# infil00p/openbts-ttsou

Measured on AMD Instinct MI355X. Metric: Mbursts/s (156.25-sym @ 4 sps) demod+detect, higher is better.
Workload: dtype f32

## Files before the change

openbts-ttsou_amd/csrc/trxsig_corr.h:

```cpp
#pragma once
#include "trxsig_dev.h"

namespace {

template <int SPS>
struct CorrGeom {
  static constexpr int NL = 36 * SPS;
  static constexpr int NC = (NL + 15) / 16;
  static constexpr int FRONT = 8 * SPS;
  static constexpr int WPAD0 = NC * 16 + 15 * SPS + 1;
  static constexpr int WPAD = ((WPAD0 + 15) / 32) * 32 + 16;
  static constexpr int H = (5 * SPS + 1 > 12) ? 5 * SPS + 1 : 12;
  static constexpr int NS = 2 * H + 1;
  static constexpr int NE = 20 * SPS;
  static constexpr int NEQ = (NE + 15) / 16;
  static constexpr int NPAIR = (NS + 2) / 2;
};
template <typename T>
__device__ __forceinline__ T &rec_slot(T *rec, int Bpad, int s, int b) { return rec[2 * ((size_t)(s >> 1) * Bpad + b) + (s & 1)]; }

template <int N>
__device__ __forceinline__ float add_row_shl(float acc, float v) {
  float r;
  if (N == 0) asm volatile("v_add_f32 %0, %1, %2" : "=v"(r) : "v"(v), "v"(acc));
  else asm volatile("v_add_f32_dpp %0, %1, %2 row_shl:%3 row_mask:0xf bank_mask:0xf bound_ctrl:1"
                    : "=v"(r) : "v"(v), "v"(acc), "n"(N));
  return r;
}
template <int SPS, int I>
__device__ __forceinline__ float energy_chain_step(float acc, const float (&nrm)[CorrGeom<SPS>::NEQ]) {
  if constexpr (I < CorrGeom<SPS>::NE) {
    acc = add_row_shl<I % 16>(acc, nrm[I / 16]);
    return energy_chain_step<SPS, I + 1>(acc, nrm);
  } else {
    return acc;
  }
}
template <int SPS, int I>
__device__ __forceinline__ float energy_chain(float acc, const float (&nrm)[CorrGeom<SPS>::NEQ]) {
  asm volatile("s_nop 1");
  return energy_chain_step<SPS, I>(acc, nrm);
}

template <int SPS>
struct CorrIn {
  typedef CorrGeom<SPS> G;
  static constexpr int NW = (CorrGeom<SPS>::NL + 15) / 16;
  cx w[NW];
  cx e[CorrGeom<SPS>::NEQ];
  int b;
  bool live, good;
  __device__ __forceinline__ void stage_window(cx *W, int r) const {
#pragma unroll
    for (int i = 0; i < NW; i++) {
      const int q = r + 16 * i;
      if (q < G::NL) W[G::FRONT + q] = w[i];
    }
  }
  __device__ __forceinline__ void stage_norms(float *ef, int r) const {
#pragma unroll
    for (int q = 0; q < G::NEQ; q++) {
      const int i = r + 16 * q;
      if (i < G::NE) ef[i] = norm2(e[q]);
    }
  }
};

template <int SPS>
__device__ __forceinline__ void corr_issue(CorrIn<SPS> &in, int b, int B, int r, const cx *__restrict__ samples,
                                           const int32_t *__restrict__ offset, const int32_t *__restrict__ length) {
  typedef CorrGeom<SPS> G;
  in.b = b;
  in.live = b < B;
  int off = 0, len = 0;
  if (in.live) { off = offset[b]; len = length[b]; }
  in.good = in.live && (off >= 0) && (len >= 92 * SPS) && (len <= 157 * SPS) && (len % SPS == 0);
  const cx *x = samples + (in.good ? off : 0);
#pragma unroll
  for (int i = 0; i < CorrIn<SPS>::NW; i++) {
    const int q = r + 16 * i;
    in.w[i] = (in.good && q < G::NL) ? x[56 * SPS + q] : mk(0, 0);
  }
#pragma unroll
  for (int q = 0; q < G::NEQ; q++) {
    const int i = r + 16 * q;
    in.e[q] = (in.good && i < G::NE) ? x[i] : mk(0, 0);
  }
}

template <int SPS, bool REC, bool EFIRST = false, unsigned TAPCLS = TRX_TAPS_GENERIC, typename IN = CorrIn<SPS>>
__device__ __forceinline__ void corr_round(const IN &in, cx *W, float4 *E, int lane, int r, const cx (&tap)[16],
                                           cx *__restrict__ rec, int Bpad, int &M_out, float &energy_out) {
  typedef CorrGeom<SPS> G;
  auto stage_norms = [&] { in.stage_norms(reinterpret_cast<float *>(E), r); };
  auto sum_norms = [&] {
    float energy = 0.0f;
#pragma unroll
    for (int i4 = 0; i4 < (G::NE + 3) / 4; i4++) {
      const float4 e = E[i4];
      energy = energy + e.x;
      if (4 * i4 + 1 < G::NE) energy = energy + e.y;
      if (4 * i4 + 2 < G::NE) energy = energy + e.z;
      if (4 * i4 + 3 < G::NE) energy = energy + e.w;
    }
    return energy;
  };
  float energy = 0.0f;
  if (EFIRST) {
    stage_norms();
    wave_lds_fence();
    energy = sum_norms();
    asm volatile("" : "+v"(energy));
    wave_lds_fence();
  }
  for (int q = r; q < G::FRONT; q += 16) W[q] = mk(0, 0);
  for (int q = G::FRONT + G::NL + r; q < G::WPAD; q += 16) W[q] = mk(0, 0);
  in.stage_window(W, r);
  if (!EFIRST) stage_norms();
  wave_lds_fence();
  if (!EFIRST) energy = sum_norms();

  float bestP = 0.0f;
  int bestT = -1;
  cx cval[G::NC];
  constexpr int CG = (SPS == 4) ? TRX_CORR_CG : 1;
  constexpr int UPC = 16 / SPS;
  constexpr int NU = UPC * (CG - 1) + 16;
#pragma unroll
  for (int c0 = 0; c0 < G::NC; c0 += CG) {
    cx sv[NU];
#pragma unroll
    for (int u = 0; u < NU; u++) sv[u] = W[r + 16 * c0 + SPS * u];
#pragma unroll
    for (int cc = 0; cc < CG; cc++) {
      if (c0 + cc < G::NC) {
        cx acc = mk(0, 0);
#pragma unroll
        for (int k = 15; k >= 0; k--) acc = cadd(acc, cmul_tap(sv[UPC * cc + k], tap[k], (TAPCLS >> (2 * k)) & 3));
        cval[c0 + cc] = acc;
      }
    }
  }
  wave_lds_fence();
#pragma unroll
  for (int c = 0; c < G::NC; c++) {
    const int t = r + 16 * c;
    if (t < G::NL) {
      W[t] = cval[c];
      const float p = norm2(cval[c]);
      if (p > bestP) { bestP = p; bestT = t; }
    }
  }
#pragma unroll
  for (int m = 1; m < 16; m <<= 1) {
    const float oP = __shfl_xor(bestP, m, 64);
    const int oT = __shfl_xor(bestT, m, 64);
    const bool take = (oP > bestP) || (oP == bestP && oT >= 0 && (bestT < 0 || oT < bestT));
    if (take) { bestP = oP; bestT = oT; }
  }
  wave_lds_fence();

  M_out = bestT;
  energy_out = energy;
  if (REC && in.live) {
    const int M = bestT;
    auto slot = [&](int s) {
      cx v = mk(0, 0);
      if (s < G::NS) {
        const int lag = M - G::H + s;
        if (lag >= 0 && lag < G::NL) v = W[lag];
      } else if (s == G::NS) {
        v = mk(__int_as_float(in.good ? M : -2), energy);
      }
      return v;
    };
    for (int j = r; j < G::NPAIR; j += 16) {
      const cx a = slot(2 * j), c = slot(2 * j + 1);
      reinterpret_cast<float4 *>(rec)[(size_t)j * Bpad + in.b] = make_float4(a.r, a.i, c.r, c.i);
    }
  }
  wave_lds_fence();
  (void)lane;
}


inline unsigned tap_classes(const TrxTables *hT, int tsc) {
  unsigned m = 0;
  for (int k = 0; k < 16; k++) {
    const trx_c32 a = hT->mid_ctap[tsc][k];
    const unsigned c = (a.r == 1.0f || a.r == -1.0f) ? 1u : ((a.i == 1.0f || a.i == -1.0f) ? 2u : 0u);
    m |= c << (2 * k);
  }
  return m;
}

}
```

openbts-ttsou_amd/csrc/trxsig_dev.h:

```cpp
#pragma once
#include <hip/hip_runtime.h>
#include <hip/hip_fp16.h>
#include <stdint.h>

#include <type_traits>

#include "trxsig_tables.h"
#include "trxsig_launch.h"

#ifndef TRX_CORR_CG
#define TRX_CORR_CG 3
#endif
#ifndef TRX_CORR_WPS
#define TRX_CORR_WPS 1
#endif
#ifndef TRX_CORR_ROUNDS
#define TRX_CORR_ROUNDS 1
#endif
#ifndef TRX_DEMOD_WAVES
#define TRX_DEMOD_WAVES 4
#endif

namespace {

typedef trx_c32 cx;

__device__ __forceinline__ cx mk(float r, float i) { cx z; z.r = r; z.i = i; return z; }
__device__ __forceinline__ cx cmul(cx x, cx a) { return mk(x.r * a.r - x.i * a.i, x.r * a.i + x.i * a.r); }
__device__ __forceinline__ cx cmul_sum(cx x, cx a, float nai) { return mk(x.r * a.r + x.i * nai, x.r * a.i + x.i * a.r); }
__device__ __forceinline__ float neg_opaque(float v) {
  float r = -v;
  asm volatile("" : "+v"(r));
  return r;
}
__device__ __forceinline__ cx cmul_sum(cx x, cx a) { return cmul_sum(x, a, neg_opaque(a.i)); }
__device__ __forceinline__ cx cmulr(cx x, float a) { return mk(x.r * a, x.i * a); }
__device__ __forceinline__ cx cadd(cx x, cx a) { return mk(x.r + a.r, x.i + a.i); }
__device__ __forceinline__ float norm2(cx x) { return x.i * x.i + x.r * x.r; }
__device__ __forceinline__ cx cinv(cx x) { float n = norm2(x); return mk(x.r / n, -x.i / n); }
__device__ __forceinline__ cx cdiv(cx x, cx a) { return cmul(x, cinv(a)); }

template <int CTRL>
__device__ __forceinline__ float dpp_f(float v) {
  return __int_as_float(__builtin_amdgcn_update_dpp(0, __float_as_int(v), CTRL, 0xf, 0xf, true));
}
template <int CTRL>
__device__ __forceinline__ int dpp_i(int v) { return __builtin_amdgcn_update_dpp(0, v, CTRL, 0xf, 0xf, true); }
__device__ __forceinline__ float wave_sum_any_order(float v) {
  v += dpp_f<0xB1>(v);
  v += dpp_f<0x4E>(v);
  v += dpp_f<0x141>(v);
  v += dpp_f<0x140>(v);
  const float r0 = __int_as_float(__builtin_amdgcn_readlane(__float_as_int(v), 0));
  const float r1 = __int_as_float(__builtin_amdgcn_readlane(__float_as_int(v), 16));
  const float r2 = __int_as_float(__builtin_amdgcn_readlane(__float_as_int(v), 32));
  const float r3 = __int_as_float(__builtin_amdgcn_readlane(__float_as_int(v), 48));
  return ((r0 + r1) + r2) + r3;
}
__device__ __forceinline__ void argmax_take(float &P, int &T, float oP, int oT) {
  const bool take = (oP > P) || (oP == P && oT >= 0 && (T < 0 || oT < T));
  P = take ? oP : P;
  T = take ? oT : T;
}
__device__ __forceinline__ void wave_argmax(float &P, int &T) {
  argmax_take(P, T, dpp_f<0xB1>(P), dpp_i<0xB1>(T));
  argmax_take(P, T, dpp_f<0x4E>(P), dpp_i<0x4E>(T));
  argmax_take(P, T, dpp_f<0x141>(P), dpp_i<0x141>(T));
  argmax_take(P, T, dpp_f<0x140>(P), dpp_i<0x140>(T));
  float bp = __int_as_float(__builtin_amdgcn_readlane(__float_as_int(P), 0));
  int bt = __builtin_amdgcn_readlane(T, 0);
#pragma unroll
  for (int r = 16; r < 64; r += 16)
    argmax_take(bp, bt, __int_as_float(__builtin_amdgcn_readlane(__float_as_int(P), r)), __builtin_amdgcn_readlane(T, r));
  P = bp; T = bt;
}

typedef float v2f __attribute__((ext_vector_type(2)));
__device__ __forceinline__ v2f pk(cx z) { v2f v = {z.r, z.i}; return v; }
__device__ __forceinline__ v2f pk_cmul(v2f x, v2f a) {
  v2f p, q, r;
  asm("v_pk_mul_f32 %0, %1, %2 op_sel_hi:[0,1]" : "=v"(p) : "v"(x), "v"(a));
  asm("v_pk_mul_f32 %0, %1, %2 op_sel:[1,1] op_sel_hi:[1,0]" : "=v"(q) : "v"(x), "v"(a));
  asm("v_pk_add_f32 %0, %1, %2 neg_lo:[0,1]" : "=v"(r) : "v"(p), "v"(q));
  return r;
}
__device__ __forceinline__ v2f pk_mul(v2f x, v2f a) {
  v2f r;
  asm("v_pk_mul_f32 %0, %1, %2" : "=v"(r) : "v"(x), "v"(a));
  return r;
}
template <int HI>
__device__ __forceinline__ v2f pk_mul_tap(v2f x, v2f t) {
  v2f r;
  if (HI) asm("v_pk_mul_f32 %0, %1, %2 op_sel:[0,1] op_sel_hi:[1,1]" : "=v"(r) : "v"(x), "v"(t));
  else asm("v_pk_mul_f32 %0, %1, %2 op_sel_hi:[1,0]" : "=v"(r) : "v"(x), "v"(t));
  return r;
}
__device__ __forceinline__ v2f pk_csub(v2f x, v2f a) {
  v2f r;
  asm("v_pk_add_f32 %0, %1, %2 neg_lo:[0,1] neg_hi:[0,1]" : "=v"(r) : "v"(x), "v"(a));
  return r;
}
__device__ __forceinline__ cx unpk(v2f v) { return mk(v.x, v.y); }
__device__ __forceinline__ v2f pk_cadd(v2f x, v2f a) {
  v2f r;
  asm("v_pk_add_f32 %0, %1, %2" : "=v"(r) : "v"(x), "v"(a));
  return r;
}

struct SmpC32 {
  static constexpr int kBytes = 8;
  static __device__ __forceinline__ cx ld(const void *base, long long i) { return reinterpret_cast<const cx *>(base)[i]; }
  typedef cx raw_t;
  static __device__ __forceinline__ raw_t ldraw(const void *base, long long i) { return reinterpret_cast<const cx *>(base)[i]; }
  static __device__ __forceinline__ raw_t zero() { return mk(0, 0); }
  static __device__ __forceinline__ cx widen(raw_t r) { return r; }
  static __device__ __forceinline__ float4 ld2(const void *base, long long first, int q) {
    return reinterpret_cast<const float4 *>(reinterpret_cast<const cx *>(base) + first)[q];
  }
};
struct SmpF16 {
  static constexpr int kBytes = 4;
  static __device__ __forceinline__ cx ld(const void *base, long long i) {
    const float2 v = __half22float2(reinterpret_cast<const __half2 *>(base)[i]);
    return mk(v.x, v.y);
  }
  typedef unsigned raw_t;
  static __device__ __forceinline__ raw_t ldraw(const void *base, long long i) { return reinterpret_cast<const unsigned *>(base)[i]; }
  static __device__ __forceinline__ raw_t zero() { return 0u; }
  static __device__ __forceinline__ cx widen(raw_t r) {
    const float2 v = __half22float2(*reinterpret_cast<const __half2 *>(&r));
    return mk(v.x, v.y);
  }
  static __device__ __forceinline__ float4 ld2(const void *base, long long first, int q) {
    const uint2 u = reinterpret_cast<const uint2 *>(reinterpret_cast<const __half2 *>(base) + first)[q];
    const float2 a = __half22float2(*reinterpret_cast<const __half2 *>(&u.x)), b = __half22float2(*reinterpret_cast<const __half2 *>(&u.y));
    return make_float4(a.x, a.y, b.x, b.y);
  }
};

struct TapArg { float v[32]; };

#define TRX_TAPS_GENERIC 0u
template <int SPS> struct TapPattern {
  static constexpr unsigned value = (SPS == 4) ? 0x19999999u : 0x99999999u;
};
__device__ __forceinline__ float fma_steer(float a, float b, float c) {
  float r;
  asm("v_fma_f32 %0, %1, %2, %3 ; steering" : "=v"(r) : "v"(a), "v"(b), "v"(c));
  return r;
}
__device__ __forceinline__ float fma_steer_s(float a, float b_sgpr, float c) {
  float r;
  asm("v_fma_f32 %0, %1, %2, %3 ; steering" : "=v"(r) : "v"(a), "s"(b_sgpr), "v"(c));
  return r;
}
__device__ __forceinline__ cx cmul_tap(cx x, cx a, int cls) {
  if (cls == 1) {
    const float p = x.i * a.i, q = x.r * a.i;
    cx z;
    asm("v_fma_f32 %0, %2, %4, -%5 ; exact-product\n\tv_fma_f32 %1, %3, %4, %6 ; exact-product"
        : "=&v"(z.r), "=v"(z.i) : "v"(x.r), "v"(x.i), "s"(a.r), "v"(p), "v"(q));
    return z;
  }
  if (cls == 2) {
    const float p = x.r * a.r, q = x.i * a.r;
    cx z;
    asm("v_fma_f32 %0, %3, -%4, %5 ; exact-product\n\tv_fma_f32 %1, %2, %4, %6 ; exact-product"
        : "=&v"(z.r), "=v"(z.i) : "v"(x.r), "v"(x.i), "s"(a.i), "v"(p), "v"(q));
    return z;
  }
  return cmul(x, a);
}

#define TRX_PI_F 3.14159274101257324f
#define TRX_2PI_F 6.28318548202514648f

template <int N>
__device__ __forceinline__ float row_shl(float v) {
  if (N == 0) return v;
  return __int_as_float(__builtin_amdgcn_update_dpp(0, __float_as_int(v), 0x100 + N, 0xf, 0xf, true));
}

__device__ __forceinline__ void lds_barrier() {
  asm volatile("s_waitcnt lgkmcnt(0)\n\ts_barrier" ::: "memory");
}
__device__ __forceinline__ void wave_lds_fence() {
  __builtin_amdgcn_fence(__ATOMIC_RELEASE, "wavefront");
  __builtin_amdgcn_wave_barrier();
  __builtin_amdgcn_fence(__ATOMIC_ACQUIRE, "wavefront");
}

__device__ __forceinline__ float dev_range_reduce(float arg) {
  if (arg > 1.0F) arg = arg - (ceilf(arg) - 1.0F);
  if (arg < 0.0F) arg = arg + ceilf(-arg);
  return arg;
}
__device__ __forceinline__ float dev_sin_lookup(const float *__restrict__ sinT, float x) {
  const float arg = dev_range_reduce(x * (1 / TRX_2PI_F));
  const float argT = arg * (float)TRX_TABLESIZE;
  int argI = (int)argT;
  argI = argI < 0 ? 0 : (argI > TRX_TABLESIZE ? TRX_TABLESIZE : argI);
  const float delta = argT - argI;
  const float iDelta = 1.0F - delta;
  return iDelta * sinT[argI] + delta * sinT[argI + 1];
}
#define TRX_FSHIFT_MAXPHASE 25000.0f
__device__ __forceinline__ cx dev_expj_lookup(const TrxTables *__restrict__ T, float x) {
  const float arg = dev_range_reduce(x * (1 / TRX_2PI_F));
  const float argT = arg * (float)TRX_TABLESIZE;
  int argI = (int)argT;
  argI = argI < 0 ? 0 : (argI > TRX_TABLESIZE ? TRX_TABLESIZE : argI);
  const float delta = argT - argI;
  const float iDelta = 1.0F - delta;
  return mk(iDelta * T->cosT[argI] + delta * T->cosT[argI + 1], iDelta * T->sinT[argI] + delta * T->sinT[argI + 1]);
}
__device__ __forceinline__ float dev_sinc(const float *__restrict__ sinT, float x) {
  if ((x >= 0.01F) || (x <= -0.01F)) return dev_sin_lookup(sinT, x) / x;
  return 1.0F;
}

}
```

openbts-ttsou_amd/csrc/trxsig_normal.hip:

```cpp
#include "trxsig_bisect.h"
#include "trxsig_corr.h"
#include "trxsig_demod.h"
#include "trxsig_rxgen.h"

#ifndef TRX_RXC_WPS
#define TRX_RXC_WPS 1
#endif
#ifndef TRX_RXD_WPS
#define TRX_RXD_WPS 1
#endif

namespace {

template <int SPS, unsigned TAPCLS>
__global__ __launch_bounds__(256, TRX_CORR_WPS) void k_tsc_corr(const TrxTables *__restrict__ T,
                                                  const cx *__restrict__ samples,
                                                  const int32_t *__restrict__ offset,
                                                  const int32_t *__restrict__ length, int B, TapArg taps,
                                                  cx *__restrict__ rec, int Bpad) {
  typedef CorrGeom<SPS> G;
  static_assert(8 * G::WPAD >= 4 * G::NE, "the energy norms are staged in the row itself");
  __shared__ __attribute__((aligned(16))) cx rows[16][G::WPAD];
  (void)T;
  const int lane = threadIdx.x & 63, wave = threadIdx.x >> 6;
  const int row = lane >> 4, r = lane & 15;
  const int slot = wave * 4 + row;

  cx tap[16];
#pragma unroll
  for (int k = 0; k < 16; k++) tap[k] = mk(taps.v[2 * k], taps.v[2 * k + 1]);

  typedef CorrIn<SPS> In;
  In in[TRX_CORR_ROUNDS];
#pragma unroll
  for (int i = 0; i < TRX_CORR_ROUNDS; i++)
    corr_issue<SPS>(in[i], (blockIdx.x * TRX_CORR_ROUNDS + i) * 16 + slot, B, r, samples, offset, length);
#pragma unroll
  for (int i = 0; i < TRX_CORR_ROUNDS; i++) {
    int M;
    float energy;
    corr_round<SPS, true, true, TAPCLS, In>(in[i], rows[slot], reinterpret_cast<float4 *>(rows[slot]), lane, r, tap, rec, Bpad, M, energy);
  }
}


#ifdef TRX_TUNING_BUILD
template <int SPS>
__global__ __launch_bounds__(64) void k_tsc_peak(const TrxTables *__restrict__ T,
                                                 const cx *__restrict__ rec, int Bpad, int B, int tsc,
                                                 float detect_thresh, float energy_thresh,
                                                 uint8_t *__restrict__ flags, cx *__restrict__ amp_out,
                                                 float *__restrict__ toa_out,
                                                 float *__restrict__ avgpwr_out) {
  typedef CorrGeom<SPS> G;
  __shared__ cx loc[26][64];
  __shared__ float pw[G::NS][64];
  const int lane = threadIdx.x;
  const int b = blockIdx.x * 64 + lane;
  const bool live = b < B;
  const int bb = live ? b : B - 1;

  const cx meta = rec_slot(rec, Bpad, G::NS, bb);
  const int M = __float_as_int(meta.r);
  const float energy = meta.i;
  const bool good = M != -2;
#pragma unroll
  for (int s = 0; s < G::NS; s++) {
    const cx v = rec_slot(rec, Bpad, s, bb);
    pw[s][lane] = norm2(v);
    const int j = s - (G::H - 12);
    if (j >= 0 && j < 24) {
      const int lag = M - 12 + j;
      loc[j][lane] = (lag > G::NL - 2) ? mk(0, 0) : v;
    }
  }
  loc[24][lane] = mk(0, 0);
  loc[25][lane] = mk(0, 0);

  float peakIx;
  const cx peak = peak_bisect<64>(T->sinc_grid, loc, lane, M, &peakIx);

  float toa = peakIx;
  cx amp = peak;
  bool detected = false;
  const bool energy_ok = good && (energy_thresh < 0.0f ||
                                  energy / (float)(unsigned)G::NE > energy_thresh * energy_thresh);
  if (!(toa < 0.0f) && !(toa > (float)G::NL) && good) {
    const int p = (int)rintf(toa);
    float valley = 0.0f;
    int numRms = 0;
#pragma unroll
    for (int i = 2 * SPS; i <= 5 * SPS; i++) {
      const int lo = p - i, hi = p + i;
      int slo = lo - M + G::H, shi = hi - M + G::H;
      slo = slo < 0 ? 0 : slo; shi = shi > G::NS - 1 ? G::NS - 1 : shi;
      const float vlo = pw[slo][lane], vhi = pw[shi][lane];
      if (lo >= 0) { valley += vlo; numRms++; }
      if (hi < G::NL) { valley += vhi; numRms++; }
    }
    if (numRms < 2) {
      amp = mk(0, 0);
    } else {
      const float RMS = (float)((double)sqrtf(valley / (float)numRms) + 0.00001);
      const float peakToMean = sqrtf(norm2(amp)) / RMS;
      amp = cdiv(amp, T->mid_gain[tsc]);
      toa = toa - T->mid_toa[tsc];
      toa = toa - (float)((66 - 56) * SPS);
      detected = peakToMean > detect_thresh;
    }
  } else {
    amp = mk(0, 0);
  }
  if (!energy_ok) { amp = mk(0, 0); toa = 0.0f; detected = false; }

  if (live) {
    uint8_t fl = 0;
    if (!good) fl = TRXSIG_F_BADLEN;
    else fl = (energy_ok ? TRXSIG_F_ENERGY : 0) | (detected ? TRXSIG_F_DETECT : 0);
    flags[b] = fl;
    amp_out[b] = amp;
    toa_out[b] = toa;
    if (avgpwr_out) avgpwr_out[b] = good ? energy / (float)(unsigned)G::NE : 0.0f;
  }
}


template <int SPS>
struct Peak8Geom {
  typedef CorrGeom<SPS> G;
  static constexpr int NV = 2 * (3 * SPS + 1);
  static constexpr int O_PW = 26 * 2;
  static constexpr int O_V = O_PW + ((G::NS + 3) & ~3);
  static constexpr int STRIDE = O_V + ((NV + 3) & ~3);
};

template <int SPS>
__global__ __launch_bounds__(256, 8) void k_tsc_peak8(const TrxTables *__restrict__ T, const cx *__restrict__ rec, int Bpad,
                                                   int B, cx gain_inv, float mid_toa, float detect_thresh,
                                                   float energy_thresh, uint8_t *__restrict__ flags,
                                                   cx *__restrict__ amp_out, float *__restrict__ toa_out,
                                                   float *__restrict__ avgpwr_out) {
  typedef CorrGeom<SPS> G;
  typedef Peak8Geom<SPS> P8;
  __shared__ __attribute__((aligned(16))) float stab[32][24];
  __shared__ __attribute__((aligned(16))) float scratch[32][P8::STRIDE];
  {
    float tv[3];
#pragma unroll
    for (int k = 0; k < 3; k++) { const int ix = threadIdx.x * 3 + k; tv[k] = T->sinc_grid[16 * (ix / 24)][ix % 24]; }
#pragma unroll
    for (int k = 0; k < 3; k++) { const int ix = threadIdx.x * 3 + k; stab[ix / 24][ix % 24] = tv[k]; }
  }
  const int lane = threadIdx.x & 63;
  const int r = lane & 7;
  const int slot = threadIdx.x >> 3;
  const int b = blockIdx.x * 32 + slot;
  const bool live = b < B;
  const int bb = live ? b : B - 1;
  float *S = scratch[slot];
  cx *loc = reinterpret_cast<cx *>(S);
  float *pw = S + P8::O_PW, *V = S + P8::O_V;

  const cx meta = rec_slot(rec, Bpad, G::NS, bb);
  const int M = __float_as_int(meta.r);
  const float energy = meta.i;
  const bool good = M != -2;
#pragma unroll
  for (int s0 = 0; s0 < G::NS; s0 += 8) {
    const int sl = s0 + r;
    if (sl < G::NS) {
      const cx v = rec_slot(rec, Bpad, sl, bb);
      pw[sl] = norm2(v);
      const int j = sl - (G::H - 12);
      if (j >= 0 && j < 24) loc[j] = (M - 12 + j > G::NL - 2) ? mk(0, 0) : v;
    }
  }
  if (r < 2) loc[24 + r] = mk(0, 0);
  __syncthreads();

  int e = 0;
  asm volatile("" : "+v"(e));
  bool active = true;
  cx peak = mk(0, 0);
  {
    const int rel2 = kFusedRel2.v[r], rel1 = kFusedRel1.v[r];
#pragma unroll
    for (int st = 0; st < 4; st++) {
      const int inc_last = 128 >> (2 * st);
      const int el = e + (rel2 >> 2) * inc_last;
      float srow[24];
      if (st < 3) {
        const float4 *rw = reinterpret_cast<const float4 *>(stab[(el & 511) >> 4]);
#pragma unroll
        for (int q = 0; q < 6; q++) {
          const float4 t4 = rw[q];
          srow[4 * q] = t4.x; srow[4 * q + 1] = t4.y; srow[4 * q + 2] = t4.z; srow[4 * q + 3] = t4.w;
        }
      } else {
        fused_row(T, el, srow);
      }
      const cx pt = fused_point(loc, el, rel2 & 3, srow);
      fused_decide<8, 2, false>(pt, lane, 2 * inc_last, e, active, peak);
    }
    {
      float srow[24];
      fused_row(T, e, srow);
      const cx pt = fused_point(loc, e, rel1 & 3, srow);
      fused_decide<8, 1, false>(pt, lane, 1, e, active, peak);
    }
    float srow[24];
    fused_row(T, e, srow);
    peak = fused_point(loc, e, 1, srow);
    asm volatile("" : "+v"(peak.r), "+v"(peak.i));
  }
  cx amp;
  float toa;
  bool detected, energy_ok;
  fused_tail<SPS, 8>([&](int lag) { const int sl = lag - M + G::H; return (sl < 0 || sl >= G::NS) ? 0.0f : pw[sl]; }, V, r, M, e,
                     peak, good, energy, gain_inv, mid_toa, detect_thresh, energy_thresh, amp, toa, detected, energy_ok);
  if (live && r == 0) {
    uint8_t fl = 0;
    if (!good) fl = TRXSIG_F_BADLEN;
    else fl = (energy_ok ? TRXSIG_F_ENERGY : 0) | (detected ? TRXSIG_F_DETECT : 0);
    flags[b] = fl;
    amp_out[b] = amp;
    toa_out[b] = toa;
    if (avgpwr_out) avgpwr_out[b] = good ? energy / (float)(unsigned)G::NE : 0.0f;
  }
}



#endif

#ifndef TRX_PEAK2_THREADS
#define TRX_PEAK2_THREADS 512
#endif
constexpr int kPeak2Threads = TRX_PEAK2_THREADS;
template <int SPS>
__global__ __launch_bounds__(kPeak2Threads) void k_tsc_peak2(const TrxTables *__restrict__ T, const cx *__restrict__ rec, int Bpad,
                                                   int B, cx gain_inv, float mid_toa, float detect_thresh,
                                                   float energy_thresh, uint8_t *__restrict__ flags,
                                                   cx *__restrict__ amp_out, float *__restrict__ toa_out,
                                                   float *__restrict__ avgpwr_out) {
  typedef CorrGeom<SPS> G;
  constexpr int NL = G::NL, NE = G::NE, NP = 3 * SPS + 3;
  __shared__ __attribute__((aligned(16))) SincLds stab;
  const int tid = threadIdx.x;
  const int h = tid & 1;
  const int b = blockIdx.x * (kPeak2Threads / 2) + (tid >> 1);
  const bool live = b < B;
  const int bb = live ? b : B - 1;
#ifdef TRX_PEAK_PROBE
  long long pt_[16] = {0};
  int pk_ = 0;
#define TRX_STAMP() pt_[pk_++] = clock64()
#else
#define TRX_STAMP()
#endif
  TRX_STAMP();

  float4 tv[3072 / kPeak2Threads];
  sinc_lds_issue<kPeak2Threads>(T, tid, tv);
  const cx meta = rec_slot(rec, Bpad, G::NS, bb);
  const int M = __float_as_int(meta.r);
  const float energy = meta.i;
  const bool good = M != -2;
  const float4 *rec4 = reinterpret_cast<const float4 *>(rec);
  cx q[23];
  {
    constexpr int S0 = G::H - 12, P0 = S0 >> 1;
    float4 pw[12];
#pragma unroll
    for (int i = 0; i < 12; i++) pw[i] = rec4[(size_t)(P0 + h + i) * Bpad + bb];
#pragma unroll
    for (int k = 0; k < 23; k++) {
      const int ix = k + 2 * h;
      const float4 p4 = pw[((S0 + k) >> 1) - P0];
      const cx v = ((S0 + k) & 1) ? mk(p4.z, p4.w) : mk(p4.x, p4.y);
      q[k] = (M - 12 + ix > NL - 2) ? mk(0, 0) : v;
    }
  }
  cx vmine_[NP];
  constexpr int VLO = G::H - (5 * SPS + 1), VHI = G::H + (2 * SPS - 1);
  if constexpr ((VLO & 1) == 0 && (VHI & 1) == 0) {
    float4 pv[(NP + 1) / 2];
#pragma unroll
    for (int i = 0; i < (NP + 1) / 2; i++) pv[i] = rec4[(size_t)(((h ? VHI : VLO) >> 1) + i) * Bpad + bb];
#pragma unroll
    for (int k = 0; k < NP; k++) vmine_[k] = (k & 1) ? mk(pv[k >> 1].z, pv[k >> 1].w) : mk(pv[k >> 1].x, pv[k >> 1].y);
  } else {
#pragma unroll
    for (int k = 0; k < NP; k++) vmine_[k] = rec_slot(rec, Bpad, (h ? VHI : VLO) + k, bb);
  }
  sinc_lds_store<kPeak2Threads>(stab, tid, tv);
  TRX_STAMP();
  __syncthreads();
  TRX_STAMP();

  int e;
  const cx peak = pair_bisect(stab, q, h, e);
  TRX_STAMP();
  const float early = (float)(M - 1) + (float)e * 0.001953125f;
  float toa = early + 1.0f;
  cx amp = peak;
  bool detected = false;
  const bool energy_ok = good && (energy_thresh < 0.0f || energy / (float)(unsigned)NE > energy_thresh * energy_thresh);
  const bool sane = !(toa < 0.0f) && !(toa > (float)NL) && good;
  if (sane) {
    const int pk = (int)rintf(toa);
    const int a = pk - M + 1;
    float plo[NP], phi[NP];
#pragma unroll
    for (int k = 0; k < NP; k++) {
      const float mine = norm2(vmine_[k]);
      const float other = __int_as_float(__builtin_amdgcn_update_dpp(0, __float_as_int(mine), 0xB1, 0xf, 0xf, true));
      plo[k] = h ? other : mine; phi[k] = h ? mine : other;
    }
    float valley = 0.0f;
#pragma unroll
    for (int i = 2 * SPS; i <= 5 * SPS; i++) {
      const int t = 5 * SPS - i, u = i - 2 * SPS;
      const float vlo = a == 0 ? plo[t] : (a == 1 ? plo[t + 1] : plo[t + 2]);
      const float vhi = a == 0 ? phi[u] : (a == 1 ? phi[u + 1] : phi[u + 2]);
      valley = valley + vlo;
      valley = valley + vhi;
    }
    int nlo = (pk < 5 * SPS ? pk : 5 * SPS) - 2 * SPS + 1;
    int nhi = (NL - 1 - pk < 5 * SPS ? NL - 1 - pk : 5 * SPS) - 2 * SPS + 1;
    nlo = nlo < 0 ? 0 : nlo; nhi = nhi < 0 ? 0 : nhi;
    const int numRms = nlo + nhi;
    if (numRms < 2) {
      amp = mk(0, 0);
    } else {
      const float RMS = (float)((double)sqrtf(valley / (float)numRms) + 0.00001);
      const float peakToMean = sqrtf(norm2(amp)) / RMS;
      amp = cmul(amp, gain_inv);
      toa = toa - mid_toa;
      toa = toa - (float)((66 - 56) * SPS);
      detected = peakToMean > detect_thresh;
    }
  } else {
    amp = mk(0, 0);
  }
  if (!energy_ok) { amp = mk(0, 0); toa = 0.0f; detected = false; }

  if (live && h == 0) {
    uint8_t fl = 0;
    if (!good) fl = TRXSIG_F_BADLEN;
    else fl = (energy_ok ? TRXSIG_F_ENERGY : 0) | (detected ? TRXSIG_F_DETECT : 0);
    flags[b] = fl;
    amp_out[b] = amp;
    toa_out[b] = toa;
    if (avgpwr_out) avgpwr_out[b] = good ? energy / (float)(unsigned)G::NE : 0.0f;
  }
#ifdef TRX_PEAK_PROBE
  TRX_STAMP();
  if (live && avgpwr_out) {
    long long v = 0;
    for (int k = 1; k < 16; k++) if ((b & 15) == k) v = pt_[k] - pt_[0];
    if (h == 0) avgpwr_out[b] = (float)v;
  }
#endif
#undef TRX_STAMP
}

template <int SPS, unsigned TAPCLS>
__global__ __launch_bounds__(256, TRX_RXC_WPS) void k_tsc_corr_rx(TrxRxGen a, int B, TapArg taps, cx *__restrict__ rec, int Bpad) {
  static_assert(SPS == 4, "the fused front end is the 260 : 96 resampler");
  typedef CorrGeom<SPS> G;
  constexpr int XCAP = 160;
  static_assert(G::WPAD >= XCAP, "the raw stretch is parked in the burst's own row");
  __shared__ __attribute__((aligned(16))) cx rows[16][G::WPAD];
  __shared__ float4 tpb_s[RXG_NT];
  if (threadIdx.x < RXG_NT) tpb_s[threadIdx.x] = a.tpb[threadIdx.x];
  __syncthreads();
  const int lane = threadIdx.x & 63, wave = threadIdx.x >> 6;
  const int row = lane >> 4, r = lane & 15;
  const int slot = wave * 4 + row;
  cx tap[16];
#pragma unroll
  for (int k = 0; k < 16; k++) tap[k] = mk(taps.v[2 * k], taps.v[2 * k + 1]);
  const int b = blockIdx.x * 16 + slot;
  CorrIn<SPS> in;
  in.b = b; in.live = b < B; in.good = in.live;
  const RxBurst u = rx_burst(a, in.live ? b : 0);
  const int jlo = rx_index(u.g0, a.skipD).j0 - 3;
  cx *X = rows[slot];
  {
    short2 v[XCAP / 16];
#pragma unroll
    for (int i = 0; i < XCAP / 16; i++) v[i] = rx_raw(a, u.s, jlo + r + 16 * i);
#pragma unroll
    for (int i = 0; i < XCAP / 16; i++) X[r + 16 * i] = rx_widen(a, v[i]);
  }
  wave_lds_fence();
  {
    static_assert(G::NL % 16 == 0 && G::NE % 16 == 0, "every lane owns a sample in every round");
    const int nb = rx_boundary(u.g0);
    RxIdx ix = rx_index(u.g0 + 56 * SPS + r, a.skipD);
#pragma unroll
    for (int i = 0; i < CorrIn<SPS>::NW; i++) {
      in.w[i] = rx_sample(X, tpb_s, jlo, ix, nb - (56 * SPS + r + 16 * i), a.w0, a.w1);
      ix = rx_step<16>(ix);
      if (i % 3 == 2) asm volatile("" : "+v"(in.w[i].r), "+v"(in.w[i].i), "+v"(in.w[i - 1].r), "+v"(in.w[i - 1].i), "+v"(in.w[i - 2].r), "+v"(in.w[i - 2].i) : : "memory");
    }
    ix = rx_index(u.g0 + r, a.skipD);
#pragma unroll
    for (int q = 0; q < G::NEQ; q++) {
      in.e[q] = rx_sample(X, tpb_s, jlo, ix, nb - (r + 16 * q), a.w0, a.w1);
      ix = rx_step<16>(ix);
      if (q % 3 == 2) asm volatile("" : "+v"(in.e[q].r), "+v"(in.e[q].i), "+v"(in.e[q - 1].r), "+v"(in.e[q - 1].i), "+v"(in.e[q - 2].r), "+v"(in.e[q - 2].i) : : "memory");
    }
  }
  wave_lds_fence();
  int M;
  float energy;
  corr_round<SPS, true, true, TAPCLS>(in, rows[slot], reinterpret_cast<float4 *>(rows[slot]), lane, r, tap, rec, Bpad, M, energy);
}

template <int SPS, bool TOL = false>
__global__ __launch_bounds__(64 * TRX_DEMOD_WAVES, TRX_RXD_WPS) void k_demod_rx(const TrxTables *__restrict__ T, TrxRxGen a, int B,
                                                                  const cx *__restrict__ amp_in, const float *__restrict__ toa_in,
                                                                  const uint8_t *__restrict__ flags, int need_mask,
                                                                  float *__restrict__ soft, uint8_t *__restrict__ hard, int nsoft,
                                                                  int stride) {
  static_assert(SPS == 4, "the fused front end is the 260 : 96 resampler");
  typedef DemodGeom<SPS, 148> G;
  constexpr int XCAP = 256;
  static_assert(G::U >= XCAP, "the raw stretch is parked in the burst's staging area");
  __shared__ cx ph[TRX_DEMOD_WAVES][G::U];
  __shared__ float4 tpb_s[RXG_NT];
  if (threadIdx.x < RXG_NT) tpb_s[threadIdx.x] = a.tpb[threadIdx.x];
  __syncthreads();
  const int lane = threadIdx.x & 63;
  const int wave = __builtin_amdgcn_readfirstlane(threadIdx.x >> 6);
  const int b = blockIdx.x * TRX_DEMOD_WAVES + wave;
  if (b >= B) return;
  float *sb = soft + (size_t)b * stride;
  uint8_t *hb = hard ? hard + (size_t)b * stride : nullptr;
  const cx amp = amp_in[b];
  const float toa = toa_in[b];
  bool enabled = fabsf(toa) <= 4096.0f;
  if (flags) enabled = enabled && (need_mask ? ((flags[b] & need_mask) == need_mask) : (flags[b] != 0));
  if (!enabled) {
    for (int m = lane; m < nsoft; m += 64) { sb[m] = 0.0f; if (hb) hb[m] = 0; }
    return;
  }
  const RxBurst u = rx_burst(a, b);
  const int jlo = rx_index(u.g0, a.skipD).j0 - 3;
  cx *X = ph[wave];
  {
    short2 v[XCAP / 64];
#pragma unroll
    for (int i = 0; i < XCAP / 64; i++) v[i] = rx_raw(a, u.s, jlo + lane + 64 * i);
#pragma unroll
    for (int i = 0; i < XCAP / 64; i++) X[lane + 64 * i] = rx_widen(a, v[i]);
  }
  wave_lds_fence();
  constexpr int NSL = (157 * SPS + 63) / 64;
  cx sv[NSL];
  {
    const int nb = rx_boundary(u.g0);
    RxIdx ix = rx_index(u.g0 + lane, a.skipD);
#pragma unroll
    for (int i = 0; i < NSL; i++) {
      sv[i] = rx_sample(X, tpb_s, jlo, ix, nb - (lane + 64 * i), a.w0, a.w1);
      ix = rx_step<64>(ix);
      if (i % 2 == 1) asm volatile("" : "+v"(sv[i].r), "+v"(sv[i].i), "+v"(sv[i - 1].r), "+v"(sv[i - 1].i) : : "memory");
    }
  }
  const int N = u.N;
  auto stage = [&](cx *P, cx inv, int lo) {
    typedef DemodGeom<SPS, 148> D;
    const int u0 = lane + lo;
    if (u0 >= 0) {
      cx *p0 = P + (u0 % SPS) * D::QLEN + u0 / SPS;
#pragma unroll
      for (int i = 0; i < NSL; i++)
        if (lane + 64 * i < N && u0 + 64 * i < D::U) p0[i * (64 / SPS)] = cmul(sv[i], inv);
    } else {
#pragma unroll
      for (int i = 0; i < NSL; i++) {
        const int uu = u0 + 64 * i;
        if (lane + 64 * i < N && uu >= 0 && uu < D::U) P[(uu % SPS) * D::QLEN + uu / SPS] = cmul(sv[i], inv);
      }
    }
  };
  if (TOL) {
    float xm = 0.0f;
#pragma unroll
    for (int i = 0; i < NSL; i++)
      if (lane + 64 * i < N) xm = max3_abs(sv[i].r, sv[i].i, xm);
    auto stage_raw = [&](cx *P, int lo) {
      typedef DemodGeom<SPS, 148> D;
      const int u0 = lane + lo;
      if (u0 >= 0) {
        cx *p0 = P + (u0 % SPS) * D::QLEN + u0 / SPS;
#pragma unroll
        for (int i = 0; i < NSL; i++)
          if (lane + 64 * i < N && u0 + 64 * i < D::U) p0[i * (64 / SPS)] = sv[i];
      } else {
#pragma unroll
        for (int i = 0; i < NSL; i++) {
          const int uu = u0 + 64 * i;
          if (lane + 64 * i < N && uu >= 0 && uu < D::U) P[(uu % SPS) * D::QLEN + uu / SPS] = sv[i];
        }
      }
    };
    if (fused_demod_tol_ex<SPS>(T, ph[wave], N, amp, toa, lane, sb, hb, nsoft, xm, stage_raw)) return;
  }
  fused_demod_ex<SPS, 64>(T, ph[wave], N, amp, toa, lane, sb, hb, nsoft, stage, [] {}, nullptr, nullptr);
}

}

int trx_rec_slots(int sps) {
  switch (sps) {
    case 1: return 2 * CorrGeom<1>::NPAIR;
    case 2: return 2 * CorrGeom<2>::NPAIR;
    case 4: return 2 * CorrGeom<4>::NPAIR;
  }
  return 0;
}

template <int S>
static void launch_tsc_detect(hipStream_t st, const TrxTables *dT, const TrxTables *hT, const trx_c32 *samples, const int32_t *off,
                              const int32_t *len, int B, int tsc, float detect_thresh, float energy_thresh,
                              trx_c32 *rec, int Bpad, uint8_t *flags, trx_c32 *amp, float *toa, float *avgpwr,
                              int variant, TrxProfiler *prof) {
  TapArg ta;
  for (int k = 0; k < 16; k++) { ta.v[2 * k] = hT->mid_ctap[tsc][k].r; ta.v[2 * k + 1] = hT->mid_ctap[tsc][k].i; }
  if (prof) prof->begin(TRXSIG_K_TSC_CORR, st);
  const dim3 cgrid((B + 16 * TRX_CORR_ROUNDS - 1) / (16 * TRX_CORR_ROUNDS));
  if (!(variant & 1) && tap_classes(hT, tsc) == TapPattern<S>::value)
    k_tsc_corr<S, TapPattern<S>::value><<<cgrid, dim3(256), 0, st>>>(dT, samples, off, len, B, ta, rec, Bpad);
  else
    k_tsc_corr<S, TRX_TAPS_GENERIC><<<cgrid, dim3(256), 0, st>>>(dT, samples, off, len, B, ta, rec, Bpad);
  if (prof) { prof->end(TRXSIG_K_TSC_CORR, st); prof->begin(TRXSIG_K_TSC_PEAK, st); }
  const trx_c32 g = hT->mid_gain[tsc];
  const float n = g.i * g.i + g.r * g.r;
  trx_c32 ginv; ginv.r = g.r / n; ginv.i = -g.i / n;
#ifdef TRX_TUNING_BUILD
  if (variant & 4) {
    k_tsc_peak<S><<<dim3((B + 63) / 64), dim3(64), 0, st>>>(dT, rec, Bpad, B, tsc, detect_thresh, energy_thresh,
                                                            flags, amp, toa, avgpwr);
  } else if (variant & 2) {
    k_tsc_peak8<S><<<dim3((B + 31) / 32), dim3(256), 0, st>>>(dT, rec, Bpad, B, ginv, hT->mid_toa[tsc], detect_thresh,
                                                              energy_thresh, flags, amp, toa, avgpwr);
  } else
#endif
  {
    k_tsc_peak2<S><<<dim3((B + kPeak2Threads / 2 - 1) / (kPeak2Threads / 2)), dim3(kPeak2Threads), 0, st>>>(dT, rec, Bpad, B, ginv, hT->mid_toa[tsc], detect_thresh,
                                                                energy_thresh, flags, amp, toa, avgpwr);
  }
  if (prof) prof->end(TRXSIG_K_TSC_PEAK, st);
}

namespace {
__global__ __launch_bounds__(256) void k_copy_verdict(const uint8_t *__restrict__ f, const cx *__restrict__ a, const float *__restrict__ t, int B,
                                                      uint8_t *__restrict__ fo, cx *__restrict__ ao, float *__restrict__ to) {
  const int b = blockIdx.x * 256 + threadIdx.x;
  if (b >= B) return;
  fo[b] = f[b]; ao[b] = a[b]; to[b] = t[b];
}
}
hipError_t trx_launch_copy_verdict(hipStream_t st, const uint8_t *flags, const trx_c32 *amp, const float *toa, int B, uint8_t *flags_out,
                                   trx_c32 *amp_out, float *toa_out) {
  if (B <= 0) return hipSuccess;
  k_copy_verdict<<<dim3((B + 255) / 256), dim3(256), 0, st>>>(flags, amp, toa, B, flags_out, amp_out, toa_out);
  return hipGetLastError();
}

hipError_t trx_launch_tsc_detect(hipStream_t st, int sps, const TrxTables *dT, const TrxTables *hT, const trx_c32 *samples,
                                 const int32_t *off, const int32_t *len, int B, int tsc,
                                 float detect_thresh, float energy_thresh, trx_c32 *rec, int Bpad,
                                 uint8_t *flags, trx_c32 *amp, float *toa, float *avgpwr, int variant,
                                 TrxProfiler *prof) {
  if (B <= 0) return hipSuccess;
  switch (sps) {
    case 1: launch_tsc_detect<1>(st, dT, hT, samples, off, len, B, tsc, detect_thresh, energy_thresh, rec, Bpad, flags, amp, toa, avgpwr, variant, prof); break;
    case 2: launch_tsc_detect<2>(st, dT, hT, samples, off, len, B, tsc, detect_thresh, energy_thresh, rec, Bpad, flags, amp, toa, avgpwr, variant, prof); break;
    case 4: launch_tsc_detect<4>(st, dT, hT, samples, off, len, B, tsc, detect_thresh, energy_thresh, rec, Bpad, flags, amp, toa, avgpwr, variant, prof); break;
    default: return hipErrorInvalidValue;
  }
  return hipGetLastError();
}

hipError_t trx_launch_rx_normal(hipStream_t st, const TrxTables *dT, const TrxTables *hT, const TrxRxGen &gen, int B, int tsc,
                                float detect_thresh, float energy_thresh, trx_c32 *rec, int Bpad, uint8_t *flags, trx_c32 *amp,
                                float *toa, float *avgpwr, float *soft, uint8_t *hard, int nsoft, int stride, int generic_taps,
                                TrxProfiler *prof, int soft_tolerance) {
  if (B <= 0) return hipSuccess;
  if (nsoft > 148 || gen.nb <= 0) return hipErrorInvalidValue;
  constexpr int S = 4;
  TapArg ta;
  for (int k = 0; k < 16; k++) { ta.v[2 * k] = hT->mid_ctap[tsc][k].r; ta.v[2 * k + 1] = hT->mid_ctap[tsc][k].i; }
  if (prof) prof->begin(TRXSIG_K_TSC_CORR, st);
  const dim3 cgrid((B + 15) / 16);
  if (!generic_taps && tap_classes(hT, tsc) == TapPattern<S>::value)
    k_tsc_corr_rx<S, TapPattern<S>::value><<<cgrid, dim3(256), 0, st>>>(gen, B, ta, rec, Bpad);
  else
    k_tsc_corr_rx<S, TRX_TAPS_GENERIC><<<cgrid, dim3(256), 0, st>>>(gen, B, ta, rec, Bpad);
  if (prof) { prof->end(TRXSIG_K_TSC_CORR, st); prof->begin(TRXSIG_K_TSC_PEAK, st); }
  const trx_c32 g = hT->mid_gain[tsc];
  const float n = g.i * g.i + g.r * g.r;
  trx_c32 ginv; ginv.r = g.r / n; ginv.i = -g.i / n;
  k_tsc_peak2<S><<<dim3((B + kPeak2Threads / 2 - 1) / (kPeak2Threads / 2)), dim3(kPeak2Threads), 0, st>>>(dT, rec, Bpad, B, ginv, hT->mid_toa[tsc], detect_thresh, energy_thresh,
                                                              flags, amp, toa, avgpwr);
  if (prof) prof->end(TRXSIG_K_TSC_PEAK, st);
  if (nsoft > 0) {
    if (prof) prof->begin(TRXSIG_K_DEMOD, st);
    if (soft_tolerance)
      k_demod_rx<S, true><<<dim3((B + TRX_DEMOD_WAVES - 1) / TRX_DEMOD_WAVES), dim3(64 * TRX_DEMOD_WAVES), 0, st>>>(
          dT, gen, B, amp, toa, flags, TRXSIG_F_DETECT, soft, hard, nsoft, stride);
    else
      k_demod_rx<S><<<dim3((B + TRX_DEMOD_WAVES - 1) / TRX_DEMOD_WAVES), dim3(64 * TRX_DEMOD_WAVES), 0, st>>>(
          dT, gen, B, amp, toa, flags, TRXSIG_F_DETECT, soft, hard, nsoft, stride);
    if (prof) prof->end(TRXSIG_K_DEMOD, st);
  }
  return hipGetLastError();
}

hipError_t trx_launch_rx_demod(hipStream_t st, const TrxTables *dT, const TrxRxGen &gen, int B, const trx_c32 *amp, const float *toa,
                               const uint8_t *flags, int need_mask, float *soft, uint8_t *hard, int nsoft, int stride, TrxProfiler *prof,
                               int soft_tolerance) {
  if (B <= 0 || nsoft <= 0) return hipSuccess;
  if (nsoft > 148 || gen.nb <= 0) return hipErrorInvalidValue;
  if (prof) prof->begin(TRXSIG_K_DEMOD, st);
  if (soft_tolerance)
    k_demod_rx<4, true><<<dim3((B + TRX_DEMOD_WAVES - 1) / TRX_DEMOD_WAVES), dim3(64 * TRX_DEMOD_WAVES), 0, st>>>(dT, gen, B, amp, toa, flags,
                                                                                                                  need_mask, soft, hard, nsoft, stride);
  else
    k_demod_rx<4><<<dim3((B + TRX_DEMOD_WAVES - 1) / TRX_DEMOD_WAVES), dim3(64 * TRX_DEMOD_WAVES), 0, st>>>(dT, gen, B, amp, toa, flags, need_mask,
                                                                                                            soft, hard, nsoft, stride);
  if (prof) prof->end(TRXSIG_K_DEMOD, st);
  return hipGetLastError();
}

hipError_t trx_launch_demod(hipStream_t st, int sps, const TrxTables *dT, const trx_c32 *samples,
                            const int32_t *off, const int32_t *len, int B, const trx_c32 *amp,
                            const float *toa, const uint8_t *flags, int need_mask, float *soft,
                            uint8_t *hard, int nsoft, int stride, TrxProfiler *prof, int soft_tolerance) {
  if (B <= 0) return hipSuccess;
  const dim3 grid((B + TRX_DEMOD_WAVES - 1) / TRX_DEMOD_WAVES), block(64 * TRX_DEMOD_WAVES);
  if (prof) prof->begin(TRXSIG_K_DEMOD, st);
#define TRX_DEMOD_CASE(S)                                                                                          \
  case S:                                                                                                          \
    if (nsoft <= 148 && soft_tolerance)                                                                            \
      k_demod<S, false, 148, SmpC32, true><<<grid, block, 0, st>>>(dT, samples, off, len, B, amp, toa, flags, need_mask, soft, hard, \
                                                     nsoft, stride);                                              \
    else if (nsoft <= 148)                                                                                         \
      k_demod<S, false, 148><<<grid, block, 0, st>>>(dT, samples, off, len, B, amp, toa, flags, need_mask, soft, hard, \
                                                     nsoft, stride);                                              \
    else                                                                                                           \
      k_demod<S, false, 157><<<grid, block, 0, st>>>(dT, samples, off, len, B, amp, toa, flags, need_mask, soft, hard, \
                                                     nsoft, stride);                                              \
    break;
  switch (sps) {
    TRX_DEMOD_CASE(1)
    TRX_DEMOD_CASE(2)
    TRX_DEMOD_CASE(4)
    default: return hipErrorInvalidValue;
  }
#undef TRX_DEMOD_CASE
  if (prof) prof->end(TRXSIG_K_DEMOD, st);
  return hipGetLastError();
}
```

Before: 627.5.

## Shrink correlator LDS rows by dropping zero padding and rotating lags

For SPS=4 the correlator's shared-memory row drops the zero-padded front and back regions. Out-of-range window taps are now handled by compile-time pad checks or clamped loads. Correlation results are written back in place per group, with the first FRONT lags held in registers and stored in rotated order, and record extraction remaps lags through tight_pos. This cuts LDS per block and removes the zero-fill stores, and the launch-bounds occupancy hint is raised to 8 waves per SIMD. The tighter register budget risks spills, and the extra fences inside the loop add synchronisation.

```diff
diff --git a/openbts-ttsou_amd/csrc/trxsig_corr.h b/openbts-ttsou_amd/csrc/trxsig_corr.h
--- a/openbts-ttsou_amd/csrc/trxsig_corr.h
+++ b/openbts-ttsou_amd/csrc/trxsig_corr.h
@@ -15,6 +15,9 @@
   static constexpr int NE = 20 * SPS;
   static constexpr int NEQ = (NE + 15) / 16;
   static constexpr int NPAIR = (NS + 2) / 2;
+  static constexpr int WTIGHT = ((NL + 15) / 32) * 32 + 16;
+  static constexpr int NHELD = FRONT / 16;
+  static __device__ __forceinline__ int tight_pos(int t) { return t >= FRONT ? t - FRONT : t + (NL - FRONT); }
 };
 template <typename T>
 __device__ __forceinline__ T &rec_slot(T *rec, int Bpad, int s, int b) { return rec[2 * ((size_t)(s >> 1) * Bpad + b) + (s & 1)]; }
@@ -50,11 +53,11 @@
   cx e[CorrGeom<SPS>::NEQ];
   int b;
   bool live, good;
-  __device__ __forceinline__ void stage_window(cx *W, int r) const {
+  __device__ __forceinline__ void stage_window(cx *win, int r) const {
 #pragma unroll
     for (int i = 0; i < NW; i++) {
       const int q = r + 16 * i;
-      if (q < G::NL) W[G::FRONT + q] = w[i];
+      if (q < G::NL) win[q] = w[i];
     }
   }
   __device__ __forceinline__ void stage_norms(float *ef, int r) const {
@@ -88,10 +91,12 @@
   }
 }
 
-template <int SPS, bool REC, bool EFIRST = false, unsigned TAPCLS = TRX_TAPS_GENERIC, typename IN = CorrIn<SPS>>
+template <int SPS, bool REC, bool EFIRST = false, unsigned TAPCLS = TRX_TAPS_GENERIC, typename IN = CorrIn<SPS>, bool TIGHT = false>
 __device__ __forceinline__ void corr_round(const IN &in, cx *W, float4 *E, int lane, int r, const cx (&tap)[16],
                                            cx *__restrict__ rec, int Bpad, int &M_out, float &energy_out) {
   typedef CorrGeom<SPS> G;
+  static_assert(!TIGHT || (REC && G::FRONT % 16 == 0 && G::NL % 16 == 0),
+                "the tight row leaves the correlation rotated, and frees and fills whole groups of 16 lags");
   auto stage_norms = [&] { in.stage_norms(reinterpret_cast<float *>(E), r); };
   auto sum_norms = [&] {
     float energy = 0.0f;
@@ -113,42 +118,86 @@
     asm volatile("" : "+v"(energy));
     wave_lds_fence();
   }
-  for (int q = r; q < G::FRONT; q += 16) W[q] = mk(0, 0);
-  for (int q = G::FRONT + G::NL + r; q < G::WPAD; q += 16) W[q] = mk(0, 0);
-  in.stage_window(W, r);
+  if (!TIGHT) {
+    for (int q = r; q < G::FRONT; q += 16) W[q] = mk(0, 0);
+    for (int q = G::FRONT + G::NL + r; q < G::WPAD; q += 16) W[q] = mk(0, 0);
+  }
+  in.stage_window(TIGHT ? W : W + G::FRONT, r);
   if (!EFIRST) stage_norms();
   wave_lds_fence();
   if (!EFIRST) energy = sum_norms();
 
   float bestP = 0.0f;
   int bestT = -1;
-  cx cval[G::NC];
   constexpr int CG = (SPS == 4) ? TRX_CORR_CG : 1;
   constexpr int UPC = 16 / SPS;
   constexpr int NU = UPC * (CG - 1) + 16;
-#pragma unroll
-  for (int c0 = 0; c0 < G::NC; c0 += CG) {
-    cx sv[NU];
-#pragma unroll
-    for (int u = 0; u < NU; u++) sv[u] = W[r + 16 * c0 + SPS * u];
-#pragma unroll
-    for (int cc = 0; cc < CG; cc++) {
-      if (c0 + cc < G::NC) {
-        cx acc = mk(0, 0);
-#pragma unroll
-        for (int k = 15; k >= 0; k--) acc = cadd(acc, cmul_tap(sv[UPC * cc + k], tap[k], (TAPCLS >> (2 * k)) & 3));
-        cval[c0 + cc] = acc;
-      }
-    }
-  }
-  wave_lds_fence();
-#pragma unroll
-  for (int c = 0; c < G::NC; c++) {
-    const int t = r + 16 * c;
-    if (t < G::NL) {
-      W[t] = cval[c];
-      const float p = norm2(cval[c]);
-      if (p > bestP) { bestP = p; bestT = t; }
+  if constexpr (TIGHT) {
+    auto pad = [](int lo) { return lo + 15 < 0 || lo >= G::NL; };
+    cx held[G::NHELD];
+#pragma unroll
+    for (int c0 = 0; c0 < G::NC; c0 += CG) {
+      cx sv[NU];
+#pragma unroll
+      for (int u = 0; u < NU; u++) {
+        const int lo = 16 * c0 + SPS * u - G::FRONT;
+        if (pad(lo)) {
+          sv[u] = mk(0, 0);
+        } else if (lo >= 0 && lo + 15 < G::NL) {
+          sv[u] = W[r + lo];
+        } else {
+          const int q = r + lo;
+          const cx v = W[q < 0 ? 0 : (q > G::NL - 1 ? G::NL - 1 : q)];
+          sv[u] = (q >= 0 && q < G::NL) ? v : mk(0, 0);
+        }
+      }
+      wave_lds_fence();
+#pragma unroll
+      for (int cc = 0; cc < CG; cc++) {
+        const int c = c0 + cc;
+        if (c < G::NC) {
+          cx acc = mk(0, 0);
+#pragma unroll
+          for (int k = 15; k >= 0; k--)
+            if (!pad(16 * c + SPS * k - G::FRONT)) acc = cadd(acc, cmul_tap(sv[UPC * cc + k], tap[k], (TAPCLS >> (2 * k)) & 3));
+          asm volatile("" : "+v"(acc.r), "+v"(acc.i) : : "memory");
+          const int t = r + 16 * c;
+          const float p = norm2(acc);
+          if (p > bestP) { bestP = p; bestT = t; }
+          if (c < G::NHELD) held[c] = acc;
+          else W[t - G::FRONT] = acc;
+        }
+      }
+      wave_lds_fence();
+    }
+#pragma unroll
+    for (int c = 0; c < G::NHELD; c++) W[G::tight_pos(r + 16 * c)] = held[c];
+  } else {
+    cx cval[G::NC];
+#pragma unroll
+    for (int c0 = 0; c0 < G::NC; c0 += CG) {
+      cx sv[NU];
+#pragma unroll
+      for (int u = 0; u < NU; u++) sv[u] = W[r + 16 * c0 + SPS * u];
+#pragma unroll
+      for (int cc = 0; cc < CG; cc++) {
+        if (c0 + cc < G::NC) {
+          cx acc = mk(0, 0);
+#pragma unroll
+          for (int k = 15; k >= 0; k--) acc = cadd(acc, cmul_tap(sv[UPC * cc + k], tap[k], (TAPCLS >> (2 * k)) & 3));
+          cval[c0 + cc] = acc;
+        }
+      }
+    }
+    wave_lds_fence();
+#pragma unroll
+    for (int c = 0; c < G::NC; c++) {
+      const int t = r + 16 * c;
+      if (t < G::NL) {
+        W[t] = cval[c];
+        const float p = norm2(cval[c]);
+        if (p > bestP) { bestP = p; bestT = t; }
+      }
     }
   }
 #pragma unroll
@@ -168,7 +217,7 @@
       cx v = mk(0, 0);
       if (s < G::NS) {
         const int lag = M - G::H + s;
-        if (lag >= 0 && lag < G::NL) v = W[lag];
+        if (lag >= 0 && lag < G::NL) v = W[TIGHT ? G::tight_pos(lag) : lag];
       } else if (s == G::NS) {
         v = mk(__int_as_float(in.good ? M : -2), energy);
       }
diff --git a/openbts-ttsou_amd/csrc/trxsig_dev.h b/openbts-ttsou_amd/csrc/trxsig_dev.h
--- a/openbts-ttsou_amd/csrc/trxsig_dev.h
+++ b/openbts-ttsou_amd/csrc/trxsig_dev.h
@@ -12,7 +12,10 @@
 #define TRX_CORR_CG 3
 #endif
 #ifndef TRX_CORR_WPS
-#define TRX_CORR_WPS 1
+#define TRX_CORR_WPS 8
+#endif
+#ifndef TRX_CORR_TIGHT
+#define TRX_CORR_TIGHT 1
 #endif
 #ifndef TRX_CORR_ROUNDS
 #define TRX_CORR_ROUNDS 1
diff --git a/openbts-ttsou_amd/csrc/trxsig_normal.hip b/openbts-ttsou_amd/csrc/trxsig_normal.hip
--- a/openbts-ttsou_amd/csrc/trxsig_normal.hip
+++ b/openbts-ttsou_amd/csrc/trxsig_normal.hip
@@ -13,14 +13,16 @@
 namespace {
 
 template <int SPS, unsigned TAPCLS>
-__global__ __launch_bounds__(256, TRX_CORR_WPS) void k_tsc_corr(const TrxTables *__restrict__ T,
+__global__ __launch_bounds__(256, SPS == 4 ? TRX_CORR_WPS : 1) void k_tsc_corr(const TrxTables *__restrict__ T,
                                                   const cx *__restrict__ samples,
                                                   const int32_t *__restrict__ offset,
                                                   const int32_t *__restrict__ length, int B, TapArg taps,
                                                   cx *__restrict__ rec, int Bpad) {
   typedef CorrGeom<SPS> G;
-  static_assert(8 * G::WPAD >= 4 * G::NE, "the energy norms are staged in the row itself");
-  __shared__ __attribute__((aligned(16))) cx rows[16][G::WPAD];
+  constexpr bool TIGHT = TRX_CORR_TIGHT && SPS == 4;
+  constexpr int ROW = TIGHT ? G::WTIGHT : G::WPAD;
+  static_assert(8 * ROW >= 4 * G::NE, "the energy norms are staged in the row itself");
+  __shared__ __attribute__((aligned(16))) cx rows[16][ROW];
   (void)T;
   const int lane = threadIdx.x & 63, wave = threadIdx.x >> 6;
   const int row = lane >> 4, r = lane & 15;
@@ -39,7 +41,7 @@
   for (int i = 0; i < TRX_CORR_ROUNDS; i++) {
     int M;
     float energy;
-    corr_round<SPS, true, true, TAPCLS, In>(in[i], rows[slot], reinterpret_cast<float4 *>(rows[slot]), lane, r, tap, rec, Bpad, M, energy);
+    corr_round<SPS, true, true, TAPCLS, In, TIGHT>(in[i], rows[slot], reinterpret_cast<float4 *>(rows[slot]), lane, r, tap, rec, Bpad, M, energy);
   }
 }
 
```

New measurement: 631.5 (median of 4 runs). No clear change (+0.6%).
